# 666DZY666/micronet

Hardware: NVIDIA H100
Metric: qat_step_images_per_sec (higher is better)
Workload: dtype f32 (bf16 tensor-core products of exact integer levels / exact bf16 pieces, fp32 accumulate)

## Files before the change

### include/micronet_b200.h

```cpp
#ifndef MICRONET_B200_H
#define MICRONET_B200_H

#include <stdint.h>

#ifdef __cplusplus
extern "C" {
#endif

typedef void* mnb_stream_t;

#define MNB_E_ARG (-1)
#define MNB_E_UNSUPPORTED (-2)

int mnb_version(void);
const char* mnb_last_error(void);
int64_t mnb_launch_count(void);

typedef struct {
  int32_t batch, in_c, in_h, in_w;
  int32_t out_c, ker_h, ker_w;
  int32_t stride_h, stride_w, pad_h, pad_w, dil_h, dil_w, groups;
} mnb_conv_shape;

#define MNB_ACT_DOREFA 1
// ... 111 lines not shown
                         uint32_t* pass_bits, uint8_t* argmax, mnb_stream_t stream);
int mnb_bn_sign_pool_bwd(const float* g, const uint32_t* pass_bits, const uint8_t* argmax, const float* x, int32_t batch,
                         int32_t channels, int32_t H, int32_t W, const float* mean, const float* invstd, const float* gamma,
                         int32_t training, int32_t out_shuffle_groups, float* dx, float* dgamma, float* dbeta,
                         float* dx_channel_sum, void* scratch, mnb_stream_t stream);

int mnb_maxpool2d_fwd(const float* x, int32_t batch, int32_t channels, int32_t H, int32_t W, int32_t kernel, int32_t stride,
                      int32_t pad, int32_t out_shuffle_groups, float* y, uint8_t* argmax, mnb_stream_t stream);
int mnb_maxpool2d_bwd(const float* g, const uint8_t* argmax, int32_t batch, int32_t channels, int32_t H, int32_t W,
                      int32_t kernel, int32_t stride, int32_t pad, int32_t out_shuffle_groups, float* dx,
                      mnb_stream_t stream);

int mnb_bn_sign_fwd_packed(const float* x, int32_t batch, int32_t channels, int32_t hw, const float* mean,
                           const float* invstd, const float* gamma, const float* beta, int32_t out_shuffle_groups, float* y,
                           uint32_t* pass_bits, void* x_packed, mnb_stream_t stream);

int mnb_fconv2d_plan(const mnb_conv_shape* s, int32_t wgrad, int32_t* out, int32_t n);
int mnb_fconv2d_fwd_tc(const mnb_conv_shape* s, const float* x, const float* w, const float* bias, float* y,
                       int32_t* err_flag, mnb_stream_t stream);
int mnb_fconv2d_wg_plan(const mnb_conv_shape* s, int32_t* out, int32_t n);
int mnb_fconv2d_fwd_wg(const mnb_conv_shape* s, const float* x, const float* w, const float* bias, float* y,
                       int32_t* err_flag, mnb_stream_t stream);
int64_t mnb_fconv2d_wgrad_tc_scratch_bytes(const mnb_conv_shape* s);
int64_t mnb_fconv2d_wgrad_wg_scratch_bytes(const mnb_conv_shape* s);
int mnb_fconv2d_wgrad_wg(const mnb_conv_shape* s, const float* dy, const float* x, float* dw, void* scratch,
                         int32_t* err_flag, mnb_stream_t stream);
int mnb_fconv2d_wgrad_tc(const mnb_conv_shape* s, const float* dy, const float* x, float* dw, void* scratch,
                         int32_t* err_flag, mnb_stream_t stream);

int64_t mnb_pk_act_bytes(int32_t batch, int32_t channels, int32_t h, int32_t w, int32_t terms);
// ... 181 lines not shown
```

### micronet_b200/_lib.py

```python
from __future__ import annotations

import ctypes as C
import os

import torch

_HERE = os.path.dirname(os.path.abspath(__file__))
LIB_PATH = os.path.join(_HERE, "lib", "libmicronet_b200.so")

ACT_DOREFA, ACT_IAO, ACT_SIGN = 1, 2, 3


class ConvShape(C.Structure):
    _fields_ = [(n, C.c_int32) for n in (
        "batch", "in_c", "in_h", "in_w", "out_c", "ker_h", "ker_w", "stride_h", "stride_w",
        "pad_h", "pad_w", "dil_h", "dil_w", "groups")]


class ActQParams(C.Structure):
    _fields_ = [("mode", C.c_int32), ("bits", C.c_int32), ("qmin", C.c_int32), ("qmax", C.c_int32),
                ("q_type", C.c_int32), ("scale", C.c_void_p), ("zero_point", C.c_void_p),
                ("obs_min", C.c_void_p), ("obs_max", C.c_void_p)]


# ... 80 lines not shown
    "mnb_pk_conv_plan_ex": (C.c_int, [_SHAPE, _I, _I, _I, _P, _I]),
    "mnb_pk_wgrad_plan": (C.c_int, [_SHAPE, _I, _I, _P, _I]),
    "mnb_pk_wimage_bytes": (_L, [_SHAPE, _I, _I, _I]),
    "mnb_pk_pack_weight": (C.c_int, [_SHAPE, _I, _I, _I, _P, _P, _P, _P, _P]),
    "mnb_pk_conv": (C.c_int, [_SHAPE, _I, _P, _I, _P, _I, _P, _P, C.c_float, _P, _P, C.c_float, _P, _P, _P]),
    "mnb_bn_sign_bwd_pack": (C.c_int, [_P, _P, _P, _I, _I, _I, _P, _P, _P, _P, _P, _I, _P, _I, _P, _P, _P]),
    "mnb_bn_sign_pool_bwd_pack": (C.c_int, [_P, _P, _P, _P, _I, _I, _I, _I, _P, _P, _P, _P, _P, _I, _P, _I, _P, _P]),
    "mnb_pk_conv_post": (C.c_int, [_SHAPE, _P, _I, _P, _I, _P, _P, C.c_float, _P, _P, C.POINTER(PkPost), _P, _P]),
    "mnb_pk_conv_post_plan": (C.c_int, [_SHAPE, _I, _I, _I, C.POINTER(PkPost), _P, _I]),
    "mnb_pk_conv_codes": (C.c_int, [_SHAPE, _P, _I, _P, _I, _P, _P, C.c_float, _P, _I, _P, _P, _P, _P]),
    "mnb_codes_decode": (C.c_int, [_P, _P, _I, _I, _I, _P, _P]),
    "mnb_bn_batch_stats_codes": (C.c_int, [_P, _P, _I, _I, _I, _D, _D, _P, _P, _P, _P, _P, _P]),
    "mnb_bn_sign_fwd_packed_codes": (C.c_int, [_P, _P, _I, _I, _I, _P, _P, _P, _P, _I, _P, _P, _P, _P]),
    "mnb_bn_sign_bwd_codes": (C.c_int, [_P, _P, _P, _P, _I, _I, _I, _P, _P, _P, _I, _I, _P, _P, _P, _P, _P, _P]),
    "mnb_bn_sign_pool_fwd_codes": (C.c_int, [_P, _P, _I, _I, _I, _I, _P, _P, _P, _P, _I, _P, _P, _P, _P]),
    "mnb_bn_sign_pool_bwd_codes": (C.c_int, [_P, _P, _P, _P, _P, _I, _I, _I, _I, _P, _P, _P, _I, _I, _P, _P, _P, _P, _P, _P]),
    "mnb_bn_sign_bwd_pack_codes": (C.c_int, [_P, _P, _P, _P, _I, _I, _I, _P, _P, _P, _P, _P, _I, _P, _I, _P, _P, _P]),
    "mnb_bn_sign_pool_bwd_pack_codes": (C.c_int, [_P, _P, _P, _P, _P, _I, _I, _I, _I, _P, _P, _P, _P, _P, _I, _P, _I, _P,
                                                  _P]),
    "mnb_quant_add_pack_fwd": (C.c_int, [_P, _P, _I, _I, _I, _I, _ACTQ, _I, _P, C.POINTER(PkPost), _P]),
    "mnb_pk_i8_act_bytes": (_L, [_I, _I, _I, _I]),
    "mnb_pk_i8_pack_act": (C.c_int, [_P, _I, _I, _I, _I, _ACTQ, _I, _I, _P, _P]),
    "mnb_pk_i8_conv_plan": (C.c_int, [_SHAPE, _P, _I]),
    "mnb_pk_i8_wimage_bytes": (_L, [_SHAPE]),
    "mnb_pk_i8_pack_weight": (C.c_int, [_SHAPE, _P, _P, _P]),
    "mnb_pk_i8_conv": (C.c_int, [_SHAPE, _P, _P, _P, _P, C.c_float, _P, _P, C.POINTER(PkPost), _P, _P]),
    "mnb_quant_add_pack_i8_fwd": (C.c_int, [_P, _P, _I, _I, _I, _I, _ACTQ, _I, _P, C.POINTER(PkPost), _P]),
    "mnb_bn_relu_quant_pack_i8_fwd": (C.c_int, [_P, _I, _I, _I, _P, _P, _P, _P, _ACTQ, _I, _P, _P]),
    "mnb_pk_plane_maxpool": (C.c_int, [_P, _I, _I, _I, _I, _I, _I, _I, _I, _P, _P]),
    "mnb_pk_plane_maxpool_requant": (C.c_int, [_P, _I, _I, _I, _I, _I, _I, _I, _I, _ACTQ, _ACTQ, _P, _P]),
# ... 132 lines not shown
```

### micronet_b200/csrc/mnb_common.cuh

```cuda
#pragma once
#include <cuda_runtime.h>
#include <float.h>
#include <stdint.h>

#include "../../include/micronet_b200.h"

int mnb_fail(int code, const char* fmt, ...);
void mnb_count_launches(int n);

#define MNB_REQUIRE(cond, ...)                            \
  do {                                                    \
    if (!(cond)) return mnb_fail(MNB_E_ARG, __VA_ARGS__); \
  } while (0)

#define MNB_LAUNCHED(nlaunch)                                                        \
  do {                                                                               \
    mnb_count_launches(nlaunch);                                                     \
    cudaError_t e__ = cudaGetLastError();                                            \
    if (e__ != cudaSuccess) return mnb_fail((int)e__, "%s:%d launch failed: %s", __FILE__, __LINE__, \
                                            cudaGetErrorString(e__));                \
  } while (0)

static inline int mnb_ceil_div(int64_t a, int64_t b) { return (int)((a + b - 1) / b); }
constexpr int MNB_NUM_SMS = 132;
// ... 26 lines not shown
  __syncthreads();
  if (lane == 0) smem[wid] = v;
  __syncthreads();
  const int nw = (blockDim.x + 31) >> 5;
  T r = (lane < nw) ? smem[lane] : identity;
  r = mnb_warp_reduce(r, op);
  return r;
}
struct MnbMin { template <typename T> __device__ T operator()(T a, T b) const { return a < b ? a : b; } };
struct MnbMax { template <typename T> __device__ T operator()(T a, T b) const { return a > b ? a : b; } };
struct MnbSum { template <typename T> __device__ T operator()(T a, T b) const { return a + b; } };

__device__ __forceinline__ float bn_bwd_centre(float g, float db, float xhat, float dg) {
  return fmaf(-xhat, dg, __fsub_rn(g, db));
}

struct XDec { float s, b; };
template <typename XT> struct XVec;
template <> struct XVec<float> { typedef float t1; typedef float2 t2; typedef float4 t4; };
template <> struct XVec<int16_t> { typedef short t1; typedef short2 t2; typedef short4 t4; };

template <typename XT>
__device__ __forceinline__ XDec x_dec(const float* dec, int channels, int c) {
  if constexpr (sizeof(XT) == 4) return XDec{1.f, 0.f};
  else return XDec{__ldg(dec + c), __ldg(dec + channels + c)};
}
template <typename XT>
__device__ __forceinline__ float x_val(XT q, XDec d) {
  if constexpr (sizeof(XT) == 4) return q;
  else return fmaf((float)q, d.s, d.b);
// ... 198 lines not shown
```

### micronet_b200/csrc/mnb_conv_packed.cu

```cuda
#include <cuda_bf16.h>

#include <algorithm>

#include "mnb_common.cuh"

namespace tcpacked {

template <int VEC> struct VecT;
template <> struct VecT<1> { typedef float type; };
template <> struct VecT<2> { typedef float2 type; };
template <> struct VecT<4> { typedef float4 type; };

template <int VEC>
__device__ __forceinline__ void store_vec(float* p, const float (&v)[VEC]) {
  typedef typename VecT<VEC>::type T;
  T t;
  float* f = reinterpret_cast<float*>(&t);
#pragma unroll
  for (int i = 0; i < VEC; ++i) f[i] = v[i];
  *reinterpret_cast<T*>(p) = t;
}

template <int VEC, typename XT>
__global__ void __launch_bounds__(256) bn_sign_packed_fwd_kernel(const XT* __restrict__ x, const float* __restrict__ dec,
                                                                 int batch, int channels, int hw, int sg, const float* __restrict__ mean,
                                                                 const float* __restrict__ invstd, const float* __restrict__ gamma,
                                                                 const float* __restrict__ beta, float* __restrict__ y,
                                                                 uint32_t* __restrict__ bits, uint4* __restrict__ xp) {
  constexpr int LPW = 32 / VEC;
  const int lane = threadIdx.x & 31;
  const int c8n = channels / 8, chunks = hw / (32 * VEC), cpg = channels / sg;
  const int64_t items = (int64_t)batch * c8n * chunks;
  const int64_t nwarps = ((int64_t)gridDim.x * blockDim.x) >> 5;
  for (int64_t w = ((int64_t)blockIdx.x * blockDim.x + threadIdx.x) >> 5; w < items; w += nwarps) {
    const int ch = (int)(w % chunks);
    const int64_t t = w / chunks;
    const int oc8 = (int)(t % c8n), b = (int)(t / c8n);
    const int pos = (ch * 32 + lane) * VEC;
    float v[8][VEC];
    int cc[8];
#pragma unroll
    for (int j = 0; j < 8; ++j) {
      const int oc = oc8 * 8 + j;
      cc[j] = sg > 1 ? (oc % sg) * cpg + oc / sg : oc;
      x_load<VEC>(x + ((int64_t)b * channels + cc[j]) * hw + pos, x_dec<XT>(dec, channels, cc[j]), v[j]);
    }
    uint32_t h[VEC][8];
#pragma unroll
    for (int j = 0; j < 8; ++j) {
      const int c = cc[j];
      const float mu = __ldg(mean + c), k = __ldg(gamma + c) * __ldg(invstd + c), be = __ldg(beta + c);
      uint32_t pass = 0;
      float yv[VEC];
#pragma unroll
      for (int i = 0; i < VEC; ++i) {
        const float bn = fmaf(v[j][i] - mu, k, be);
        const bool neg = bn < 0.f;
        yv[i] = neg ? -1.f : 1.f;
        h[i][j] = neg ? 0xBF80u : 0x3F80u;
        pass |= (fabsf(bn) < 1.f ? 1u : 0u) << i;
      }
      if (y) store_vec<VEC>(y + ((int64_t)b * channels + oc8 * 8 + j) * hw + pos, yv);
      uint32_t word = pass << (VEC * (lane % LPW));
#pragma unroll
      for (int o = 1; o < LPW; o <<= 1) word |= __shfl_xor_sync(0xffffffffu, word, o);
      if (lane % LPW == 0) bits[(((int64_t)b * channels + c) * hw + pos) >> 5] = word;
    }
    uint4* dst = xp + ((int64_t)b * c8n + oc8) * hw + pos;
#pragma unroll
    for (int i = 0; i < VEC; ++i)
      dst[i] = make_uint4(h[i][0] | (h[i][1] << 16), h[i][2] | (h[i][3] << 16), h[i][4] | (h[i][5] << 16), h[i][6] | (h[i][7] << 16));
  }
}

}

template <typename XT>
static int bn_sign_fwd_packed(const XT* x, const float* dec, int32_t batch, int32_t channels, int32_t hw, const float* mean,
                              const float* invstd, const float* gamma, const float* beta, int32_t out_shuffle_groups, float* y,
                              uint32_t* pass_bits, void* x_packed, mnb_stream_t stream) {
  MNB_REQUIRE(x && mean && invstd && gamma && beta && pass_bits && x_packed, "NULL bn_sign_fwd_packed pointer");
  MNB_REQUIRE(batch > 0 && channels > 0 && hw > 0, "bad bn_sign_fwd_packed shape");
  MNB_REQUIRE(out_shuffle_groups >= 1 && channels % out_shuffle_groups == 0, "shuffle groups %d do not divide %d channels",
              out_shuffle_groups, channels);
  if (channels % 8 || hw % 32 || (reinterpret_cast<uintptr_t>(x_packed) & 15))
    return mnb_fail(MNB_E_UNSUPPORTED, "packed producer needs channels %% 8 == 0, H*W %% 32 == 0, 16-byte aligned output");
// ... 33 lines not shown
```

### micronet_b200/csrc/mnb_fused.cu

```cuda
#include <algorithm>

#include "mnb_common.cuh"

static inline cudaStream_t S(mnb_stream_t s) { return (cudaStream_t)s; }
constexpr int FUSED_SPLITS = 32;

__device__ __forceinline__ uint32_t shuffled_channel(uint32_t c, uint32_t sg, uint32_t cpg) {
  return sg > 1 ? (c % cpg) * sg + c / cpg : c;
}

__global__ void __launch_bounds__(256) bn_sign_fwd_v4_kernel(const float4* __restrict__ x, uint32_t n4, uint32_t channels,
                                                             uint32_t hw4, uint32_t sg, const float* __restrict__ mean,
                                                             const float* __restrict__ invstd, const float* __restrict__ gamma,
                                                             const float* __restrict__ beta, float4* __restrict__ y,
                                                             uint32_t* __restrict__ bits) {
  const uint32_t lane = threadIdx.x & 31;
  const uint32_t stride = gridDim.x * blockDim.x;
  const uint32_t n4_up = (n4 + 31u) & ~31u;
  const uint32_t cpg = channels / sg;
  for (uint32_t i = blockIdx.x * blockDim.x + threadIdx.x; i < n4_up; i += stride) {
    uint32_t nib = 0;
    if (i < n4) {
      const uint32_t plane = i / hw4, off = i - plane * hw4;
      const uint32_t b = plane / channels, c = plane - b * channels;
// ... 312 lines not shown
      const uint32_t a1 = first_max_of_signs(pos[2], pos[3], pos[6], pos[7]);
      const float m0 = (pos[0] | pos[1] | pos[4] | pos[5]) ? 1.f : -1.f, m1 = (pos[2] | pos[3] | pos[6] | pos[7]) ? 1.f : -1.f;
      const uint32_t oplane = b * gm.channels + shuffled_channel(c, gm.sg, cpg);
      y[(oplane * gm.OH + oh) * gm.OW2 + j] = make_float2(m0, m1);
      arg[o] = make_uchar2((unsigned char)a0, (unsigned char)a1);
    }
    const uint32_t other = __shfl_xor_sync(0xffffffffu, nib, 1);
    if (live && (threadIdx.x & 1) == 0) {
      bits8[i0 >> 1] = (uint8_t)((nib & 15u) | ((other & 15u) << 4));
      bits8[(i0 + gm.W4) >> 1] = (uint8_t)((nib >> 4) | (other & 0xf0u));
    }
  }
}

template <typename XT>
__global__ void __launch_bounds__(256) bn_sign_pool_bwd_reduce_kernel(const float2* __restrict__ g, const uchar2* __restrict__ arg,
                                                                      const uint8_t* __restrict__ bits8, const XT* __restrict__ x,
                                                                      const float* __restrict__ dec, int batch, PoolGeom gm, const float* __restrict__ mean,
                                                                      const float* __restrict__ invstd, float* __restrict__ dgamma,
                                                                      float* __restrict__ dbeta, uint32_t* counters, double* partial) {
  __shared__ double red[32];
  __shared__ bool last;
  const uint32_t c = blockIdx.x, sp = blockIdx.y, nsp = gridDim.y;
  const uint32_t oc = shuffled_channel(c, gm.sg, gm.channels / gm.sg);
  const float mu = __ldg(mean + c), is = __ldg(invstd + c);
  const XDec d = x_dec<XT>(dec, (int)gm.channels, (int)c);
  const uint32_t b_lo = (uint32_t)((int64_t)batch * sp / nsp), b_hi = (uint32_t)((int64_t)batch * (sp + 1) / nsp);
  const uint32_t per_img = gm.OH * gm.OW2, total = (b_hi - b_lo) * per_img;
  float f1[2] = {0.f, 0.f}, f2[2] = {0.f, 0.f};
  for (uint32_t t0 = threadIdx.x; t0 < total; t0 += 2 * blockDim.x) {
// ... 133 lines not shown
                                    float* y, uint32_t* pass_bits, uint8_t* argmax, mnb_stream_t stream) {
  return bn_sign_pool_fwd<float>(x, nullptr, batch, channels, H, W, mean, invstd, gamma, beta, out_shuffle_groups, y, pass_bits,
                                 argmax, stream);
}

extern "C" int mnb_bn_sign_pool_fwd_codes(const int16_t* codes, const float* dec, int32_t batch, int32_t channels, int32_t H,
                                          int32_t W, const float* mean, const float* invstd, const float* gamma, const float* beta,
                                          int32_t out_shuffle_groups, float* y, uint32_t* pass_bits, uint8_t* argmax,
                                          mnb_stream_t stream) {
  MNB_REQUIRE(dec, "NULL decode pair");
  return bn_sign_pool_fwd<int16_t>(codes, dec, batch, channels, H, W, mean, invstd, gamma, beta, out_shuffle_groups, y, pass_bits,
                                   argmax, stream);
}

template <typename XT>
static int bn_sign_pool_bwd(const float* g, const uint32_t* pass_bits, const uint8_t* argmax, const XT* x, const float* dec,
                            int32_t batch, int32_t channels, int32_t H, int32_t W, const float* mean, const float* invstd,
                            const float* gamma, int32_t training, int32_t out_shuffle_groups, float* dx, float* dgamma,
                            float* dbeta, float* dx_channel_sum, void* scratch, mnb_stream_t stream) {
  MNB_REQUIRE(g && pass_bits && argmax && x && mean && invstd && gamma && dx && dgamma && dbeta && scratch,
              "NULL bn_sign_pool_bwd pointer");
  PoolGeom gm;
  if (int e = pool_geom(batch, channels, H, W, out_shuffle_groups, x, dx, nullptr, gm)) return e;
  MNB_REQUIRE((reinterpret_cast<uintptr_t>(g) & 7) == 0, "pooled gradient must be 8-byte aligned");
  const int64_t per = (int64_t)batch * H * W;
  const int splits = plane_splits(batch, per, channels);
  uint32_t* counters = reinterpret_cast<uint32_t*>(reinterpret_cast<char*>(scratch) + 16384);
  double* partial = reinterpret_cast<double*>(reinterpret_cast<char*>(scratch) + 49152);
  const dim3 grid(channels, splits);
  const uint8_t* bits8 = reinterpret_cast<const uint8_t*>(pass_bits);
// ... 207 lines not shown
```

### micronet_b200/csrc/mnb_pk.cu

```cuda
#include <cuda.h>
#include <cuda_bf16.h>

#include <algorithm>
#include <cstdlib>
#include <cstring>

#include "mnb_common.cuh"
#include "mnb_tc.cuh"

namespace pk {

constexpr int MAXST = 8;
constexpr int MAXTAP = 64, MAXTMPL = 16, MAXY = 4, MAXPAIR = 6, MAXPROG = 512;
constexpr int kSmemBudget = 227 * 1024 - 3072;
constexpr int kNtSizes[] = {16, 32, 48, 64, 96, 128};

struct Tmpl { int kph, tap0, ntap, blk_off, blk_bytes; };

struct Plan {
  int mode;
  int B, G, R, S, stride;
  int HA, WA, C8A, nkph;
  int kg, ng, NOUT;
  int OHr, OWr, OH, OW, omul, ny;
// ... 636 lines not shown
      dst = (((int64_t)bi * 4 * C8 + oct) * (H >> 1) + (h >> 1)) * (W >> 1) + (w >> 1);
    } else {
      dst = (int64_t)plane * HW + pos;
    }
    if constexpr (CPU == 16) out_pk[dst] = pack16_s8(lev);
    else out_pk[dst] = make_uint4(pack2(lev[0], lev[1]), pack2(lev[2], lev[3]), pack2(lev[4], lev[5]), pack2(lev[6], lev[7]));
  }
}

template <int VEC> struct PkVec;
template <> struct PkVec<1> { typedef float type; };
template <> struct PkVec<2> { typedef float2 type; };
template <> struct PkVec<4> { typedef float4 type; };

template <int VEC, typename XT>
__global__ void __launch_bounds__(256) bn_sign_bwd_pack_kernel(const float* __restrict__ g, const uint32_t* __restrict__ bits,
                                                               const XT* __restrict__ x, const float* __restrict__ dec,
                                                               int batch, int channels, int hw,
                                                               int sg, float inv_count, const float* __restrict__ mean,
                                                               const float* __restrict__ invstd, const float* __restrict__ gamma,
                                                               const float* __restrict__ dgamma, const float* __restrict__ dbeta,
                                                               const float* __restrict__ ch_scale, int terms,
                                                               float* __restrict__ dx, uint4* __restrict__ out, int64_t plane_vecs) {
  typedef typename PkVec<VEC>::type T;
  const int lane = threadIdx.x & 31;
  const int c8n = channels / 8, cpg = channels / sg, chunks = hw / (32 * VEC);
  const int64_t items = (int64_t)batch * c8n * chunks;
  const int64_t nwarps = ((int64_t)gridDim.x * blockDim.x) >> 5;
  for (int64_t w = ((int64_t)blockIdx.x * blockDim.x + threadIdx.x) >> 5; w < items; w += nwarps) {
    const int ch = (int)(w % chunks);
    const int64_t pl = w / chunks;
    const int c8 = (int)(pl % c8n), b = (int)(pl / c8n);
    const int pos = (ch * 32 + lane) * VEC;
    T gv[8];
    float xf[8][VEC];
    uint32_t bw[8];
#pragma unroll
    for (int j = 0; j < 8; ++j) {
      const int c = c8 * 8 + j;
// ... 11 lines not shown
      const float db = __ldg(dbeta + c) * inv_count, dg = __ldg(dgamma + c) * inv_count;
      const float sc = ch_scale ? __ldg(ch_scale + c) : 1.f;
      const float* gf = reinterpret_cast<const float*>(&gv[j]);
      T dv;
      float* df = reinterpret_cast<float*>(&dv);
#pragma unroll
      for (int i = 0; i < VEC; ++i) {
        float t = ((bw[j] >> i) & 1u) ? gf[i] : 0.f;
        t = bn_bwd_centre(t, db, (xf[j][i] - mu) * is, dg);
        t = k * t;
        df[i] = t;
        v[i][j] = ch_scale ? __fmul_rn(t, sc) : t;
      }
      if (dx) *reinterpret_cast<T*>(dx + ((int64_t)b * channels + c) * hw + pos) = dv;
    }
    const int64_t dst = pl * hw + pos;
    for (int tm = 0; tm < terms; ++tm) {
#pragma unroll
      for (int i = 0; i < VEC; ++i) {
        uint32_t pk4[4];
#pragma unroll
        for (int j = 0; j < 4; ++j) {
          pk4[j] = pack2(v[i][2 * j], v[i][2 * j + 1]);
          v[i][2 * j] -= __uint_as_float(pk4[j] << 16);
          v[i][2 * j + 1] -= __uint_as_float(pk4[j] & 0xffff0000u);
        }
        out[(int64_t)tm * plane_vecs + dst + i] = make_uint4(pk4[0], pk4[1], pk4[2], pk4[3]);
      }
    }
  }
}

template <typename XT>
__global__ void __launch_bounds__(256) bn_sign_pool_bwd_pack_kernel(const float2* __restrict__ g, const uchar2* __restrict__ arg,
                                                                    const uint8_t* __restrict__ bits8, const XT* __restrict__ x,
                                                                    const float* __restrict__ dec, int batch, int channels, int H, int W4, int sg, float inv_count,
                                                                    const float* __restrict__ mean, const float* __restrict__ invstd,
                                                                    const float* __restrict__ gamma, const float* __restrict__ dgamma,
                                                                    const float* __restrict__ dbeta, const float* __restrict__ ch_scale,
                                                                    int terms, uint4* __restrict__ out, int64_t plane_vecs) {
  const uint32_t OH = (uint32_t)H / 2u, OW2 = (uint32_t)W4, c8n = (uint32_t)channels / 8u, cpg = (uint32_t)channels / (uint32_t)sg;
  const uint32_t per_plane = OH * OW2;
  const int64_t total = (int64_t)batch * c8n * per_plane;
  for (int64_t it = (int64_t)blockIdx.x * blockDim.x + threadIdx.x; it < total; it += (int64_t)gridDim.x * blockDim.x) {
    const uint32_t rem = (uint32_t)(it % per_plane);
    const int64_t pl = it / per_plane;
    const uint32_t c8 = (uint32_t)(pl % c8n), b = (uint32_t)(pl / c8n);
    const uint32_t oh = rem / OW2, j = rem - oh * OW2;
    float v[8][8];
#pragma unroll
    for (int q = 0; q < 8; ++q) {
      const uint32_t c = c8 * 8u + q;
      const uint32_t oc = sg > 1 ? (c % cpg) * (uint32_t)sg + c / cpg : c;
      const uint32_t plane = b * (uint32_t)channels + c;
      const float2 gv = __ldg(g + ((size_t)(b * (uint32_t)channels + oc) * OH + oh) * OW2 + j);
      const uchar2 a = arg[((size_t)plane * OH + oh) * OW2 + j];
      const uint32_t i0 = (plane * (uint32_t)H + 2u * oh) * (uint32_t)W4 + j, i1 = i0 + (uint32_t)W4;
      const uint32_t n0 = (bits8[i0 >> 1] >> (4u * (i0 & 1u))) & 15u, n1 = (bits8[i1 >> 1] >> (4u * (i1 & 1u))) & 15u;
// ... 4 lines not shown
      const float sc = ch_scale ? __ldg(ch_scale + c) : 1.f;
      const uint32_t e0 = (a.x >> 1) * 4u + (a.x & 1u), e1 = (a.y >> 1) * 4u + 2u + (a.y & 1u);
      const uint32_t nib = n0 | (n1 << 4);
      const float xs[8] = {r0.x, r0.y, r0.z, r0.w, r1.x, r1.y, r1.z, r1.w};
#pragma unroll
      for (int e = 0; e < 8; ++e) {
        float t = 0.f;
        if ((uint32_t)e == e0 && ((nib >> e) & 1u)) t = gv.x;
        if ((uint32_t)e == e1 && ((nib >> e) & 1u)) t = gv.y;
        t = bn_bwd_centre(t, db, (xs[e] - mu) * is, dg);
        t = k * t;
        v[e][q] = ch_scale ? __fmul_rn(t, sc) : t;
      }
    }
    const int64_t dst0 = (pl * H + 2 * oh) * (int64_t)(4 * W4) + 4 * j;
    for (int tm = 0; tm < terms; ++tm) {
#pragma unroll
      for (int e = 0; e < 8; ++e) {
        uint32_t pk4[4];
#pragma unroll
        for (int q = 0; q < 4; ++q) {
          pk4[q] = pack2(v[e][2 * q], v[e][2 * q + 1]);
          v[e][2 * q] -= __uint_as_float(pk4[q] << 16);
          v[e][2 * q + 1] -= __uint_as_float(pk4[q] & 0xffff0000u);
        }
        out[(int64_t)tm * plane_vecs + dst0 + (e >> 2) * (int64_t)(4 * W4) + (e & 3)] = make_uint4(pk4[0], pk4[1], pk4[2], pk4[3]);
      }
    }
  }
}

struct PackWParams {
  Plan pl;
  const int16_t* w_int; const float* w_f32; const float* kzero;
  int cin_g, cout_g;
};

template <int CPU>
__global__ void __launch_bounds__(256) pack_weight_kernel(const __grid_constant__ PackWParams pp, uint4* __restrict__ out) {
  const Plan& p = pp.pl;
  const int64_t total = p.wimg_bytes / 16;
// ... 2106 lines not shown
```

### micronet_b200/csrc/mnb_quant.cu

```cuda
#include <math.h>
#include <stdarg.h>
#include <stdio.h>

#include <atomic>

#include "mnb_common.cuh"

static thread_local char g_mnb_err[512] = "";
static std::atomic<int64_t> g_mnb_launches{0};

int mnb_fail(int code, const char* fmt, ...) {
  va_list ap;
  va_start(ap, fmt);
  vsnprintf(g_mnb_err, sizeof(g_mnb_err), fmt, ap);
  va_end(ap);
  return code;
}
void mnb_count_launches(int n) { g_mnb_launches.fetch_add(n, std::memory_order_relaxed); }

extern "C" int mnb_version(void) { return 100; }
extern "C" const char* mnb_last_error(void) { return g_mnb_err; }
extern "C" int64_t mnb_launch_count(void) { return g_mnb_launches.load(); }

static inline cudaStream_t S(mnb_stream_t s) { return (cudaStream_t)s; }
// ... 574 lines not shown

template <typename XT>
__global__ void __launch_bounds__(256) channel_stats_kernel(const XT* __restrict__ x, const float* __restrict__ dec, int batch,
                                                            int channels, int hw, int as_mean_var, float* __restrict__ stats,
                                                            uint32_t* counters, double* partial, MnbBnUpdate bn) {
  __shared__ double red[32];
  __shared__ bool last;
  const int c = blockIdx.x, sp = blockIdx.y, nsp = gridDim.y;
  const int64_t per = (int64_t)batch * hw;
  double s1 = 0.0, s2 = 0.0;
  const XDec d = x_dec<XT>(dec, channels, c);
  const float pivot = as_mean_var ? x_val<XT>(__ldg(x + (int64_t)c * hw), d) : 0.f;
  const int b_lo = (int)((int64_t)batch * sp / nsp), b_hi = (int)((int64_t)batch * (sp + 1) / nsp);
  const bool vec = (hw & 3) == 0 && ((reinterpret_cast<uintptr_t>(x) & (4 * sizeof(XT) - 1)) == 0);
  if (vec) {
    const uint32_t hw4 = (uint32_t)hw >> 2, total = (uint32_t)(b_hi - b_lo) * hw4;
    float f1[4] = {0.f, 0.f, 0.f, 0.f}, f2[4] = {0.f, 0.f, 0.f, 0.f};
    for (uint32_t t0 = threadIdx.x; t0 < total; t0 += 4 * blockDim.x) {
#pragma unroll
      for (int u = 0; u < 4; ++u) {
        const uint32_t t = t0 + u * blockDim.x;
        if (t < total) {
          const uint32_t b = t / hw4, i = t - b * hw4;
          float4 v = x_load4(x + 4 * (((int64_t)(b_lo + b) * channels + c) * hw4 + i), d);
          v.x -= pivot; v.y -= pivot; v.z -= pivot; v.w -= pivot;
          f1[u] += (v.x + v.y) + (v.z + v.w);
          f2[u] += (v.x * v.x + v.y * v.y) + (v.z * v.z + v.w * v.w);
        }
      }
    }
    s1 = ((double)f1[0] + (double)f1[1]) + ((double)f1[2] + (double)f1[3]);
    s2 = ((double)f2[0] + (double)f2[1]) + ((double)f2[2] + (double)f2[3]);
  } else {
    for (int b = b_lo; b < b_hi; ++b) {
      const XT* plane = x + ((int64_t)b * channels + c) * hw;
      float f1 = 0.f, f2 = 0.f;
      for (int i = threadIdx.x; i < hw; i += blockDim.x) {
        const float v = x_val<XT>(__ldg(plane + i), d) - pivot;
        f1 += v; f2 += v * v;
      }
      s1 += (double)f1;
      s2 += (double)f2;
    }
// ... 315 lines not shown
```

### micronet_b200/fused.py

```python
from __future__ import annotations

import torch
import torch.nn as nn
from torch.autograd import Function

import ctypes as C

import torch.nn.functional as TF

from . import _lib as L
from . import pk as PK


def _xargs(lib, name, x, codes):
    if codes is None:
        return getattr(lib, name), (x.data_ptr(),)
    return getattr(lib, name + "_codes"), (codes[0].data_ptr(), codes[1].data_ptr())


class BNSignFn(Function):

    @staticmethod
    def forward(ctx, x, gamma, beta, mean, invstd, training, shuffle_groups, pool, plane_only=False):
        from . import functional as F_
        lib = L.load()
        x = x.contiguous()
        b, c = x.shape[0], x.shape[1]
        hw = x.numel() // (b * c)
        pk_conv = getattr(x, "_mnb_pk_conv", None)
        codes = getattr(x, "_mnb_codes", None)
        write_plane = L.PK_WBWTAB and c % 8 == 0 and hw % 32 == 0 and x.dim() == 4 and L.PK_MODE != "off"
        if codes is not None and not pool and not write_plane:
            x, codes = F_.materialized(x), None
        bits = torch.empty((x.numel() + 31) // 32, dtype=torch.int32, device=x.device)
        arg = None
        if pool:
            h, w = x.shape[2], x.shape[3]
            y = torch.empty((b, c, h // 2, w // 2), dtype=x.dtype, device=x.device)
            arg = torch.empty(y.numel(), dtype=torch.uint8, device=x.device)
            fn, xa = _xargs(lib, "mnb_bn_sign_pool_fwd", x, codes)
            L.check(fn(*xa, b, c, h, w, mean.data_ptr(), invstd.data_ptr(), gamma.data_ptr(), beta.data_ptr(), shuffle_groups,
                       y.data_ptr(), bits.data_ptr(), arg.data_ptr(), L.stream()), "bn_sign_pool_fwd")
        else:
            y = torch.empty_like(x)
            written = False
            if write_plane:
                plane = torch.empty(x.numel() * 2, dtype=torch.uint8, device=x.device)
                skip_y = bool(plane_only) and L.PLANE_ONLY
                fn, xa = _xargs(lib, "mnb_bn_sign_fwd_packed", x, codes)
                rc = fn(*xa, b, c, hw, mean.data_ptr(), invstd.data_ptr(), gamma.data_ptr(), beta.data_ptr(), shuffle_groups,
                        None if skip_y else y.data_ptr(), bits.data_ptr(), plane.data_ptr(), L.stream())
                if rc == 0:
                    y._mnb_pk_pm1 = plane
                    if skip_y:
                        y._mnb_plane_only = True
                    written = True
                elif rc != L.E_UNSUPPORTED:
# ... 465 lines not shown
```

Before: 41720.

## Fuse pooled BN-sign with packed plane write; stage packed stores; prefetch BN stats

Adds a pooled BN-sign forward kernel that also emits the bf16 ±1 packed plane, so the next packed conv need not repack the pooled output. Packed-plane stores in the BN-sign forward and backward-pack kernels go through a swizzled per-warp shared-memory stage, so each warp writes contiguous coalesced runs, and those kernels get launch bounds of 2 blocks per SM. The batch-stats reduction now uses incremental offsets and software prefetching of the next loads. These are several unrelated changes that add shared memory use and code complexity.

```diff
diff --git a/include/micronet_b200.h b/include/micronet_b200.h
--- a/include/micronet_b200.h
+++ b/include/micronet_b200.h
@@ -149,6 +149,13 @@
 int mnb_bn_sign_fwd_packed(const float* x, int32_t batch, int32_t channels, int32_t hw, const float* mean,
                            const float* invstd, const float* gamma, const float* beta, int32_t out_shuffle_groups, float* y,
                            uint32_t* pass_bits, void* x_packed, mnb_stream_t stream);
+int mnb_bn_sign_pool_fwd_packed(const float* x, int32_t batch, int32_t channels, int32_t H, int32_t W, const float* mean,
+                                const float* invstd, const float* gamma, const float* beta, int32_t out_shuffle_groups,
+                                float* y, uint32_t* pass_bits, uint8_t* argmax, void* x_packed, mnb_stream_t stream);
+int mnb_bn_sign_pool_fwd_packed_codes(const int16_t* codes, const float* dec, int32_t batch, int32_t channels, int32_t H,
+                                      int32_t W, const float* mean, const float* invstd, const float* gamma, const float* beta,
+                                      int32_t out_shuffle_groups, float* y, uint32_t* pass_bits, uint8_t* argmax,
+                                      void* x_packed, mnb_stream_t stream);
 
 int mnb_fconv2d_plan(const mnb_conv_shape* s, int32_t wgrad, int32_t* out, int32_t n);
 int mnb_fconv2d_fwd_tc(const mnb_conv_shape* s, const float* x, const float* w, const float* bias, float* y,
diff --git a/micronet_b200/_lib.py b/micronet_b200/_lib.py
--- a/micronet_b200/_lib.py
+++ b/micronet_b200/_lib.py
@@ -118,6 +118,8 @@
     "mnb_bn_sign_fwd_packed_codes": (C.c_int, [_P, _P, _I, _I, _I, _P, _P, _P, _P, _I, _P, _P, _P, _P]),
     "mnb_bn_sign_bwd_codes": (C.c_int, [_P, _P, _P, _P, _I, _I, _I, _P, _P, _P, _I, _I, _P, _P, _P, _P, _P, _P]),
     "mnb_bn_sign_pool_fwd_codes": (C.c_int, [_P, _P, _I, _I, _I, _I, _P, _P, _P, _P, _I, _P, _P, _P, _P]),
+    "mnb_bn_sign_pool_fwd_packed": (C.c_int, [_P, _I, _I, _I, _I, _P, _P, _P, _P, _I, _P, _P, _P, _P, _P]),
+    "mnb_bn_sign_pool_fwd_packed_codes": (C.c_int, [_P, _P, _I, _I, _I, _I, _P, _P, _P, _P, _I, _P, _P, _P, _P, _P]),
     "mnb_bn_sign_pool_bwd_codes": (C.c_int, [_P, _P, _P, _P, _P, _I, _I, _I, _I, _P, _P, _P, _I, _I, _P, _P, _P, _P, _P, _P]),
     "mnb_bn_sign_bwd_pack_codes": (C.c_int, [_P, _P, _P, _P, _I, _I, _I, _P, _P, _P, _P, _P, _I, _P, _I, _P, _P, _P]),
     "mnb_bn_sign_pool_bwd_pack_codes": (C.c_int, [_P, _P, _P, _P, _P, _I, _I, _I, _I, _P, _P, _P, _P, _P, _I, _P, _I, _P,
diff --git a/micronet_b200/csrc/mnb_common.cuh b/micronet_b200/csrc/mnb_common.cuh
--- a/micronet_b200/csrc/mnb_common.cuh
+++ b/micronet_b200/csrc/mnb_common.cuh
@@ -64,6 +64,8 @@
 __device__ __forceinline__ float bn_bwd_centre(float g, float db, float xhat, float dg) {
   return fmaf(-xhat, dg, __fsub_rn(g, db));
 }
+
+__device__ __forceinline__ uint32_t mnb_stage_slot(uint32_t u) { return (u & ~7u) | ((u ^ (u >> 3)) & 7u); }
 
 struct XDec { float s, b; };
 template <typename XT> struct XVec;
diff --git a/micronet_b200/csrc/mnb_conv_packed.cu b/micronet_b200/csrc/mnb_conv_packed.cu
--- a/micronet_b200/csrc/mnb_conv_packed.cu
+++ b/micronet_b200/csrc/mnb_conv_packed.cu
@@ -21,13 +21,21 @@
   *reinterpret_cast<T*>(p) = t;
 }
 
+__device__ __forceinline__ uint4 bf16_pm1_pixel(uint32_t neg) {
+  uint32_t w[4];
+#pragma unroll
+  for (int q = 0; q < 4; ++q) w[q] = 0x3F803F80u | (((neg >> (2 * q)) & 1u) << 15) | (((neg >> (2 * q + 1)) & 1u) << 31);
+  return make_uint4(w[0], w[1], w[2], w[3]);
+}
+
 template <int VEC, typename XT>
-__global__ void __launch_bounds__(256) bn_sign_packed_fwd_kernel(const XT* __restrict__ x, const float* __restrict__ dec,
+__global__ void __launch_bounds__(256, 2) bn_sign_packed_fwd_kernel(const XT* __restrict__ x, const float* __restrict__ dec,
                                                                  int batch, int channels, int hw, int sg, const float* __restrict__ mean,
                                                                  const float* __restrict__ invstd, const float* __restrict__ gamma,
                                                                  const float* __restrict__ beta, float* __restrict__ y,
                                                                  uint32_t* __restrict__ bits, uint4* __restrict__ xp) {
   constexpr int LPW = 32 / VEC;
+  __shared__ uint4 stage[8][32 * VEC];
   const int lane = threadIdx.x & 31;
   const int c8n = channels / 8, chunks = hw / (32 * VEC), cpg = channels / sg;
   const int64_t items = (int64_t)batch * c8n * chunks;
@@ -45,7 +53,7 @@
       cc[j] = sg > 1 ? (oc % sg) * cpg + oc / sg : oc;
       x_load<VEC>(x + ((int64_t)b * channels + cc[j]) * hw + pos, x_dec<XT>(dec, channels, cc[j]), v[j]);
     }
-    uint32_t h[VEC][8];
+    uint32_t neg = 0;
 #pragma unroll
     for (int j = 0; j < 8; ++j) {
       const int c = cc[j];
@@ -55,9 +63,8 @@
 #pragma unroll
       for (int i = 0; i < VEC; ++i) {
         const float bn = fmaf(v[j][i] - mu, k, be);
-        const bool neg = bn < 0.f;
-        yv[i] = neg ? -1.f : 1.f;
-        h[i][j] = neg ? 0xBF80u : 0x3F80u;
+        yv[i] = bn < 0.f ? -1.f : 1.f;
+        neg |= (bn < 0.f ? 1u : 0u) << (8 * i + j);
         pass |= (fabsf(bn) < 1.f ? 1u : 0u) << i;
       }
       if (y) store_vec<VEC>(y + ((int64_t)b * channels + oc8 * 8 + j) * hw + pos, yv);
@@ -66,10 +73,18 @@
       for (int o = 1; o < LPW; o <<= 1) word |= __shfl_xor_sync(0xffffffffu, word, o);
       if (lane % LPW == 0) bits[(((int64_t)b * channels + c) * hw + pos) >> 5] = word;
     }
-    uint4* dst = xp + ((int64_t)b * c8n + oc8) * hw + pos;
+    uint4* dst = xp + ((int64_t)b * c8n + oc8) * hw + ch * 32 * VEC;
+    if constexpr (VEC == 1) {
+      dst[lane] = bf16_pm1_pixel(neg);
+    } else {
+      uint4* st = stage[threadIdx.x >> 5];
 #pragma unroll
-    for (int i = 0; i < VEC; ++i)
-      dst[i] = make_uint4(h[i][0] | (h[i][1] << 16), h[i][2] | (h[i][3] << 16), h[i][4] | (h[i][5] << 16), h[i][6] | (h[i][7] << 16));
+      for (int i = 0; i < VEC; ++i) st[mnb_stage_slot(lane * VEC + i)] = bf16_pm1_pixel(neg >> (8 * i));
+      __syncwarp();
+#pragma unroll
+      for (int k = 0; k < VEC; ++k) dst[k * 32 + lane] = st[mnb_stage_slot(k * 32 + lane)];
+      __syncwarp();
+    }
   }
 }
 
diff --git a/micronet_b200/csrc/mnb_fused.cu b/micronet_b200/csrc/mnb_fused.cu
--- a/micronet_b200/csrc/mnb_fused.cu
+++ b/micronet_b200/csrc/mnb_fused.cu
@@ -350,6 +350,69 @@
 }
 
 template <typename XT>
+__global__ void __launch_bounds__(256) bn_sign_pool_fwd_plane_kernel(const XT* __restrict__ x, const float* __restrict__ dec,
+                                                                     uint32_t n_items, PoolGeom gm,
+                                                                     const float* __restrict__ mean, const float* __restrict__ invstd,
+                                                                     const float* __restrict__ gamma, const float* __restrict__ beta,
+                                                                     float2* __restrict__ y, uchar2* __restrict__ arg,
+                                                                     uint8_t* __restrict__ bits8, uint4* __restrict__ xp) {
+  const uint32_t stride = gridDim.x * blockDim.x;
+  const uint32_t n_up = (n_items + 31u) & ~31u;
+  const uint32_t cpg = gm.channels / gm.sg, c8n = gm.channels / 8u;
+  for (uint32_t it = blockIdx.x * blockDim.x + threadIdx.x; it < n_up; it += stride) {
+    const bool live = it < n_items;
+    uint32_t j = 0, oh = 0, b = 0, oc8 = 0;
+    if (live) {
+      j = it % gm.OW2;
+      const uint32_t t = it / gm.OW2;
+      oh = t % gm.OH;
+      const uint32_t pl = t / gm.OH;
+      b = pl / c8n; oc8 = pl - b * c8n;
+    }
+    uint32_t neg = 0;
+#pragma unroll 2
+    for (uint32_t q = 0; q < 8; ++q) {
+      const uint32_t oc = oc8 * 8u + q;
+      const uint32_t c = gm.sg > 1 ? (oc % gm.sg) * cpg + oc / gm.sg : oc;
+      const uint32_t plane = b * gm.channels + c;
+      const uint32_t o = (plane * gm.OH + oh) * gm.OW2 + j;
+      uint32_t nib = 0, i0 = 0;
+      if (live) {
+        i0 = (plane * gm.H + 2 * oh) * gm.W4 + j;
+        const float mu = __ldg(mean + c), sc = __ldg(gamma + c) * __ldg(invstd + c), be = __ldg(beta + c);
+        const XDec d = x_dec<XT>(dec, (int)gm.channels, (int)c);
+        const float4 r0 = x_load4(x + 4 * i0, d), r1 = x_load4(x + 4 * (i0 + gm.W4), d);
+        const float v[8] = {fmaf(r0.x - mu, sc, be), fmaf(r0.y - mu, sc, be), fmaf(r0.z - mu, sc, be), fmaf(r0.w - mu, sc, be),
+                            fmaf(r1.x - mu, sc, be), fmaf(r1.y - mu, sc, be), fmaf(r1.z - mu, sc, be), fmaf(r1.w - mu, sc, be)};
+        bool pos[8];
+#pragma unroll
+        for (int e = 0; e < 8; ++e) { pos[e] = !(v[e] < 0.f); nib |= (uint32_t)(fabsf(v[e]) < 1.f) << e; }
+        const uint32_t a0 = first_max_of_signs(pos[0], pos[1], pos[4], pos[5]);
+        const uint32_t a1 = first_max_of_signs(pos[2], pos[3], pos[6], pos[7]);
+        const bool p0 = pos[0] | pos[1] | pos[4] | pos[5], p1 = pos[2] | pos[3] | pos[6] | pos[7];
+        if (y) y[((b * gm.channels + oc) * gm.OH + oh) * gm.OW2 + j] = make_float2(p0 ? 1.f : -1.f, p1 ? 1.f : -1.f);
+        arg[o] = make_uchar2((unsigned char)a0, (unsigned char)a1);
+        neg |= ((p0 ? 0u : 1u) << q) | ((p1 ? 0u : 1u) << (8 + q));
+      }
+      const uint32_t other = __shfl_xor_sync(0xffffffffu, nib, 1);
+      if (live && (threadIdx.x & 1) == 0) {
+        bits8[i0 >> 1] = (uint8_t)((nib & 15u) | ((other & 15u) << 4));
+        bits8[(i0 + gm.W4) >> 1] = (uint8_t)((nib >> 4) | (other & 0xf0u));
+      }
+    }
+    if (live) {
+      uint4* dst = xp + ((size_t)(b * c8n + oc8) * gm.OH + oh) * (2 * gm.OW2) + 2 * j;
+      uint32_t w[8];
+#pragma unroll
+      for (int k = 0; k < 8; ++k)
+        w[k] = 0x3F803F80u | (((neg >> (2 * k)) & 1u) << 15) | (((neg >> (2 * k + 1)) & 1u) << 31);
+      dst[0] = make_uint4(w[0], w[1], w[2], w[3]);
+      dst[1] = make_uint4(w[4], w[5], w[6], w[7]);
+    }
+  }
+}
+
+template <typename XT>
 __global__ void __launch_bounds__(256) bn_sign_pool_bwd_reduce_kernel(const float2* __restrict__ g, const uchar2* __restrict__ arg,
                                                                       const uint8_t* __restrict__ bits8, const XT* __restrict__ x,
                                                                       const float* __restrict__ dec, int batch, PoolGeom gm, const float* __restrict__ mean,
@@ -513,6 +576,44 @@
 }
 
 template <typename XT>
+static int bn_sign_pool_fwd_packed(const XT* x, const float* dec, int32_t batch, int32_t channels, int32_t H, int32_t W,
+                                   const float* mean, const float* invstd, const float* gamma, const float* beta,
+                                   int32_t out_shuffle_groups, float* y, uint32_t* pass_bits, uint8_t* argmax, void* x_packed,
+                                   mnb_stream_t stream) {
+  MNB_REQUIRE(x && mean && invstd && gamma && beta && pass_bits && argmax && x_packed,
+              "NULL bn_sign_pool_fwd_packed pointer");
+  PoolGeom gm;
+  if (int e = pool_geom(batch, channels, H, W, out_shuffle_groups, x, y, nullptr, gm)) return e;
+  if (channels % 8 || (reinterpret_cast<uintptr_t>(x_packed) & 15))
+    return mnb_fail(MNB_E_UNSUPPORTED, "pooled packed producer needs channels %% 8 == 0 and a 16-byte aligned plane");
+  const uint32_t n_items = (uint32_t)((int64_t)batch * (channels / 8) * gm.OH * gm.OW2);
+  int blocks = (int)std::min<int64_t>(mnb_ceil_div(n_items, 256), MNB_NUM_SMS * 16);
+  bn_sign_pool_fwd_plane_kernel<XT><<<blocks, 256, 0, S(stream)>>>(x, dec, n_items, gm, mean, invstd, gamma, beta,
+                                                                   reinterpret_cast<float2*>(y), reinterpret_cast<uchar2*>(argmax),
+                                                                   reinterpret_cast<uint8_t*>(pass_bits),
+                                                                   reinterpret_cast<uint4*>(x_packed));
+  MNB_LAUNCHED(1);
+  return 0;
+}
+
+extern "C" int mnb_bn_sign_pool_fwd_packed(const float* x, int32_t batch, int32_t channels, int32_t H, int32_t W,
+                                           const float* mean, const float* invstd, const float* gamma, const float* beta,
+                                           int32_t out_shuffle_groups, float* y, uint32_t* pass_bits, uint8_t* argmax,
+                                           void* x_packed, mnb_stream_t stream) {
+  return bn_sign_pool_fwd_packed<float>(x, nullptr, batch, channels, H, W, mean, invstd, gamma, beta, out_shuffle_groups, y,
+                                        pass_bits, argmax, x_packed, stream);
+}
+
+extern "C" int mnb_bn_sign_pool_fwd_packed_codes(const int16_t* codes, const float* dec, int32_t batch, int32_t channels,
+                                                 int32_t H, int32_t W, const float* mean, const float* invstd,
+                                                 const float* gamma, const float* beta, int32_t out_shuffle_groups, float* y,
+                                                 uint32_t* pass_bits, uint8_t* argmax, void* x_packed, mnb_stream_t stream) {
+  MNB_REQUIRE(dec, "NULL decode pair");
+  return bn_sign_pool_fwd_packed<int16_t>(codes, dec, batch, channels, H, W, mean, invstd, gamma, beta, out_shuffle_groups, y,
+                                          pass_bits, argmax, x_packed, stream);
+}
+
+template <typename XT>
 static int bn_sign_pool_bwd(const float* g, const uint32_t* pass_bits, const uint8_t* argmax, const XT* x, const float* dec,
                             int32_t batch, int32_t channels, int32_t H, int32_t W, const float* mean, const float* invstd,
                             const float* gamma, int32_t training, int32_t out_shuffle_groups, float* dx, float* dgamma,
diff --git a/micronet_b200/csrc/mnb_pk.cu b/micronet_b200/csrc/mnb_pk.cu
--- a/micronet_b200/csrc/mnb_pk.cu
+++ b/micronet_b200/csrc/mnb_pk.cu
@@ -674,7 +674,7 @@
 template <> struct PkVec<4> { typedef float4 type; };
 
 template <int VEC, typename XT>
-__global__ void __launch_bounds__(256) bn_sign_bwd_pack_kernel(const float* __restrict__ g, const uint32_t* __restrict__ bits,
+__global__ void __launch_bounds__(256, 2) bn_sign_bwd_pack_kernel(const float* __restrict__ g, const uint32_t* __restrict__ bits,
                                                                const XT* __restrict__ x, const float* __restrict__ dec,
                                                                int batch, int channels, int hw,
                                                                int sg, float inv_count, const float* __restrict__ mean,
@@ -683,6 +683,7 @@
                                                                const float* __restrict__ ch_scale, int terms,
                                                                float* __restrict__ dx, uint4* __restrict__ out, int64_t plane_vecs) {
   typedef typename PkVec<VEC>::type T;
+  __shared__ uint4 stage[8][32 * VEC];
   const int lane = threadIdx.x & 31;
   const int c8n = channels / 8, cpg = channels / sg, chunks = hw / (32 * VEC);
   const int64_t items = (int64_t)batch * c8n * chunks;
@@ -724,7 +725,8 @@
       }
       if (dx) *reinterpret_cast<T*>(dx + ((int64_t)b * channels + c) * hw + pos) = dv;
     }
-    const int64_t dst = pl * hw + pos;
+    const int64_t run = pl * hw + ch * 32 * VEC;
+    uint4* st = stage[threadIdx.x >> 5];
     for (int tm = 0; tm < terms; ++tm) {
 #pragma unroll
       for (int i = 0; i < VEC; ++i) {
@@ -735,7 +737,15 @@
           v[i][2 * j] -= __uint_as_float(pk4[j] << 16);
           v[i][2 * j + 1] -= __uint_as_float(pk4[j] & 0xffff0000u);
         }
-        out[(int64_t)tm * plane_vecs + dst + i] = make_uint4(pk4[0], pk4[1], pk4[2], pk4[3]);
+        const uint4 px = make_uint4(pk4[0], pk4[1], pk4[2], pk4[3]);
+        if constexpr (VEC == 1) out[(int64_t)tm * plane_vecs + run + lane] = px;
+        else st[mnb_stage_slot(lane * VEC + i)] = px;
+      }
+      if constexpr (VEC > 1) {
+        __syncwarp();
+#pragma unroll
+        for (int k = 0; k < VEC; ++k) out[(int64_t)tm * plane_vecs + run + k * 32 + lane] = st[mnb_stage_slot(k * 32 + lane)];
+        __syncwarp();
       }
     }
   }
@@ -752,6 +762,8 @@
   const uint32_t OH = (uint32_t)H / 2u, OW2 = (uint32_t)W4, c8n = (uint32_t)channels / 8u, cpg = (uint32_t)channels / (uint32_t)sg;
   const uint32_t per_plane = OH * OW2;
   const int64_t total = (int64_t)batch * c8n * per_plane;
+  __shared__ uint4 stage[8][256];
+  const bool staged = per_plane % 32u == 0 && 32u % OW2 == 0;
   for (int64_t it = (int64_t)blockIdx.x * blockDim.x + threadIdx.x; it < total; it += (int64_t)gridDim.x * blockDim.x) {
     const uint32_t rem = (uint32_t)(it % per_plane);
     const int64_t pl = it / per_plane;
@@ -786,6 +798,9 @@
       }
     }
     const int64_t dst0 = (pl * H + 2 * oh) * (int64_t)(4 * W4) + 4 * j;
+    const uint32_t lane = threadIdx.x & 31u;
+    uint4* st = stage[threadIdx.x >> 5];
+    const int64_t run0 = dst0 - (int64_t)(lane / OW2) * (8 * W4) - 4 * (lane % OW2);
     for (int tm = 0; tm < terms; ++tm) {
 #pragma unroll
       for (int e = 0; e < 8; ++e) {
@@ -796,7 +811,17 @@
           v[e][2 * q] -= __uint_as_float(pk4[q] << 16);
           v[e][2 * q + 1] -= __uint_as_float(pk4[q] & 0xffff0000u);
         }
-        out[(int64_t)tm * plane_vecs + dst0 + (e >> 2) * (int64_t)(4 * W4) + (e & 3)] = make_uint4(pk4[0], pk4[1], pk4[2], pk4[3]);
+        const uint4 px = make_uint4(pk4[0], pk4[1], pk4[2], pk4[3]);
+        if (staged)
+          st[mnb_stage_slot((2u * (lane / OW2) + (e >> 2)) * 4u * OW2 + 4u * (lane % OW2) + (e & 3))] = px;
+        else
+          out[(int64_t)tm * plane_vecs + dst0 + (e >> 2) * (int64_t)(4 * W4) + (e & 3)] = px;
+      }
+      if (staged) {
+        __syncwarp();
+#pragma unroll
+        for (int k = 0; k < 8; ++k) out[(int64_t)tm * plane_vecs + run0 + k * 32 + lane] = st[mnb_stage_slot(k * 32 + lane)];
+        __syncwarp();
       }
     }
   }
diff --git a/micronet_b200/csrc/mnb_quant.cu b/micronet_b200/csrc/mnb_quant.cu
--- a/micronet_b200/csrc/mnb_quant.cu
+++ b/micronet_b200/csrc/mnb_quant.cu
@@ -612,19 +612,44 @@
   const int b_lo = (int)((int64_t)batch * sp / nsp), b_hi = (int)((int64_t)batch * (sp + 1) / nsp);
   const bool vec = (hw & 3) == 0 && ((reinterpret_cast<uintptr_t>(x) & (4 * sizeof(XT) - 1)) == 0);
   if (vec) {
+    typedef typename XVec<XT>::t4 R4;
+    const R4* xr = reinterpret_cast<const R4*>(x);
     const uint32_t hw4 = (uint32_t)hw >> 2, total = (uint32_t)(b_hi - b_lo) * hw4;
+    const size_t img = (size_t)channels * hw4;
+    const uint32_t step = 4 * blockDim.x, step_b = step / hw4, step_i = step - step_b * hw4;
+    const R4* base = xr + ((int64_t)b_lo * channels + c) * hw4;
+    size_t off[4];
+    uint32_t ii[4];
+#pragma unroll
+    for (int u = 0; u < 4; ++u) {
+      const uint32_t t = threadIdx.x + u * blockDim.x, b = t / hw4;
+      ii[u] = t - b * hw4;
+      off[u] = (size_t)b * img + ii[u];
+    }
     float f1[4] = {0.f, 0.f, 0.f, 0.f}, f2[4] = {0.f, 0.f, 0.f, 0.f};
-    for (uint32_t t0 = threadIdx.x; t0 < total; t0 += 4 * blockDim.x) {
+    R4 cur[4] = {};
+    uint32_t t0 = threadIdx.x;
+#pragma unroll
+    for (int u = 0; u < 4; ++u)
+      if (t0 + u * blockDim.x < total) cur[u] = __ldg(base + off[u]);
+    for (; t0 < total; t0 += step) {
+      R4 nxt[4] = {};
 #pragma unroll
       for (int u = 0; u < 4; ++u) {
-        const uint32_t t = t0 + u * blockDim.x;
-        if (t < total) {
-          const uint32_t b = t / hw4, i = t - b * hw4;
-          float4 v = x_load4(x + 4 * (((int64_t)(b_lo + b) * channels + c) * hw4 + i), d);
+        ii[u] += step_i;
+        off[u] += (size_t)step_b * img + step_i;
+        if (ii[u] >= hw4) { ii[u] -= hw4; off[u] += img - hw4; }
+        if (t0 + step + u * blockDim.x < total) nxt[u] = __ldg(base + off[u]);
+      }
+#pragma unroll
+      for (int u = 0; u < 4; ++u) {
+        if (t0 + u * blockDim.x < total) {
+          float4 v = make_float4(x_val<XT>(cur[u].x, d), x_val<XT>(cur[u].y, d), x_val<XT>(cur[u].z, d), x_val<XT>(cur[u].w, d));
           v.x -= pivot; v.y -= pivot; v.z -= pivot; v.w -= pivot;
           f1[u] += (v.x + v.y) + (v.z + v.w);
           f2[u] += (v.x * v.x + v.y * v.y) + (v.z * v.z + v.w * v.w);
         }
+        cur[u] = nxt[u];
       }
     }
     s1 = ((double)f1[0] + (double)f1[1]) + ((double)f1[2] + (double)f1[3]);
diff --git a/micronet_b200/fused.py b/micronet_b200/fused.py
--- a/micronet_b200/fused.py
+++ b/micronet_b200/fused.py
@@ -38,9 +38,20 @@
             h, w = x.shape[2], x.shape[3]
             y = torch.empty((b, c, h // 2, w // 2), dtype=x.dtype, device=x.device)
             arg = torch.empty(y.numel(), dtype=torch.uint8, device=x.device)
-            fn, xa = _xargs(lib, "mnb_bn_sign_pool_fwd", x, codes)
-            L.check(fn(*xa, b, c, h, w, mean.data_ptr(), invstd.data_ptr(), gamma.data_ptr(), beta.data_ptr(), shuffle_groups,
-                       y.data_ptr(), bits.data_ptr(), arg.data_ptr(), L.stream()), "bn_sign_pool_fwd")
+            rc = L.E_UNSUPPORTED
+            if L.PK_WBWTAB and c % 8 == 0 and L.PK_MODE != "off":
+                plane = torch.empty(y.numel() * 2, dtype=torch.uint8, device=x.device)
+                fn, xa = _xargs(lib, "mnb_bn_sign_pool_fwd_packed", x, codes)
+                rc = fn(*xa, b, c, h, w, mean.data_ptr(), invstd.data_ptr(), gamma.data_ptr(), beta.data_ptr(), shuffle_groups,
+                        y.data_ptr(), bits.data_ptr(), arg.data_ptr(), plane.data_ptr(), L.stream())
+                if rc == 0:
+                    y._mnb_pk_pm1 = plane
+                elif rc != L.E_UNSUPPORTED:
+                    L.check(rc, "bn_sign_pool_fwd_packed")
+            if rc != 0:
+                fn, xa = _xargs(lib, "mnb_bn_sign_pool_fwd", x, codes)
+                L.check(fn(*xa, b, c, h, w, mean.data_ptr(), invstd.data_ptr(), gamma.data_ptr(), beta.data_ptr(),
+                           shuffle_groups, y.data_ptr(), bits.data_ptr(), arg.data_ptr(), L.stream()), "bn_sign_pool_fwd")
         else:
             y = torch.empty_like(x)
             written = False
```

Result: faster. 42680 (median of 6 runs) (+2.3%).
